# neggles/neurosis

Hardware: AMD Instinct MI355X
Metric: train images/sec (node) SDXL 1024^2 (higher is better)
Workload: dtype bf16

## Files before the change

### neurosis_amd/csrc/conv_halo.h

```cpp
#pragma once
#include <type_traits>

#ifdef NK_HALO_STAMPS
__device__ unsigned long long nk_halo_stamp_buf[8 * 8192];
__device__ unsigned long long nk_halo_kstep_buf[3 * 16 * 20 * 5];
#define CH_KSTAMP(t, ph) do { const int w_ = tid >> 6; if ((tid & 63) == 0 && (w_ == 0 || w_ == 4 || w_ == 6) && blockIdx.x >= 2048 && blockIdx.x < 2048 + 16 && (t) < 20) \
    nk_halo_kstep_buf[((((w_ == 0 ? 0 : (w_ == 4 ? 1 : 2)) * 16 + (blockIdx.x - 2048)) * 20 + (t)) * 5) + (ph)] = __builtin_amdgcn_s_memtime(); } while (0)
extern "C" int nk_debug_halo_ksteps(unsigned long long* host_out) {
  return hipMemcpyFromSymbol(host_out, HIP_SYMBOL(nk_halo_kstep_buf), sizeof(nk_halo_kstep_buf)) == hipSuccess ? 0 : 1;
}
#define CH_STAMP(slot) do { if (tid == 0 && blockIdx.x < 8192) nk_halo_stamp_buf[blockIdx.x * 8 + (slot)] = __builtin_amdgcn_s_memtime(); } while (0)
#define CH_STAMP_RT(slot) do { if (tid == 0 && blockIdx.x < 8192) nk_halo_stamp_buf[blockIdx.x * 8 + (slot)] = __builtin_amdgcn_s_memrealtime(); } while (0)
extern "C" int nk_debug_halo_stamps(unsigned long long* host_out, int nwg) {
  return hipMemcpyFromSymbol(host_out, HIP_SYMBOL(nk_halo_stamp_buf), (size_t)nwg * 8 * sizeof(unsigned long long)) == hipSuccess ? 0 : 1;
}
#else
#define CH_STAMP(slot)
#define CH_STAMP_RT(slot)
#define CH_KSTAMP(t, ph)
#endif
#define CH_TW 32
#define CH_HW (CH_TW + 2)
#define CH_BSTAGE 20480
#define CH_NS 3
#define CH_BSTAGE_DEEP 16384
#define CH_NS_DEEP 4
template <int BN_> struct HaloRing {
#ifdef NK_HALO_FIRE_IN_M
  static constexpr bool DEEP = false;
#else
  static constexpr bool DEEP = BN_ == 128;
#endif
  static constexpr int BST = DEEP ? CH_BSTAGE_DEEP : CH_BSTAGE;
  static constexpr int NS = DEEP ? CH_NS_DEEP : CH_NS;
  static constexpr int AHEAD = 2;
#ifdef NK_HALO_NO_PROD
  static constexpr bool PROD = false;
#else
  static constexpr bool PROD = DEEP;
#endif
  static constexpr bool FIRE_IN_R = DEEP && !PROD;
  static constexpr int THREADS = PROD ? 768 : 512;
  static constexpr int WAVES_PER_SIMD = PROD ? 3 : 2;
};
#define CH_NPROD_W 3
#define CH_NBW 6

template <int MI>
struct HaloGeom {
  static constexpr int TH = 2 * MI;
  static constexpr int RPW = MI / 2;
  static constexpr int HPX = (TH + 2) * CH_HW;
  static constexpr int HPIECES = ((HPX + 7) / 8 + 1) & ~1;
  static constexpr int HBUF = HPIECES * 1024;
  static constexpr int HPW = HPIECES / 2;
  static constexpr int SMEM = 2 * HBUF + CH_NS * CH_BSTAGE;
  static constexpr int SMEM_DEEP = 2 * HBUF + CH_NS_DEEP * CH_BSTAGE_DEEP;
  template <int BN_> static constexpr int smem() { return HaloRing<BN_>::DEEP ? SMEM_DEEP : SMEM; }
};
constexpr int ch_count(int NPH, int LAST, int t) { return t > LAST ? 0 : (NPH + LAST - t) / (LAST + 1); }
constexpr int ch_start(int NPH, int LAST, int t) { int s = 0; for (int u = 0; u < t; ++u) s += ch_count(NPH, LAST, u); return s; }

template <int BN_, int NBW = CH_NBW>
struct HaloWeights {
  static constexpr int NPC = BN_ / 8;
  static constexpr int NPW = (NPC + NBW - 1) / NBW;
  const bf16_t* rp[NPW];
  bool ok[NPW];
  __device__ __forceinline__ static int pieces(int wave) { return wave >= NBW ? 0 : (wave + NBW * (NPW - 1) < NPC ? NPW : NPW - 1); }
  __device__ __forceinline__ void init(const bf16_t* Wt, long ld, int Cout, int n0, int wave, int lane) {
#pragma unroll
    for (int i = 0; i < NPW; ++i) {
      const int pc = wave + NBW * i;
      const int row = pc * 8 + (lane >> 3);
      const int chunk = (lane & 7) ^ (lane >> 3);
      ok[i] = wave < NBW && pc < NPC && n0 + row < Cout;
      rp[i] = Wt + (long)(n0 + (ok[i] ? row : 0)) * ld + chunk * 8;
    }
  }
  __device__ __forceinline__ void fire_next(bool live, long adv, char* img, int wave) {
    const bf16_t* zp = (const bf16_t*)nk_zero_page;
#pragma unroll
    for (int i = 0; i < NPW; ++i) {
      if (wave + NBW * i < NPC)
        __builtin_amdgcn_global_load_lds((nk_gptr)((live && ok[i]) ? rp[i] : zp), (nk_lptr)(img + (wave + NBW * i) * 1024), 16, 0, 0);
      rp[i] += adv;
    }
  }
};

template <int BN_, int MI, int STATS>
__global__ __launch_bounds__(HaloRing<BN_>::THREADS, HaloRing<BN_>::WAVES_PER_SIMD) void nk_conv3x3_halo_kernel(const NkGemmParams p) {
  extern __shared__ __attribute__((aligned(16))) char smem[];
  using G = HaloGeom<MI>;
  using R = HaloRing<BN_>;
  constexpr int HN = BN_ / 2, NJ = HN / 16;
  constexpr int RPW = G::RPW, HPW = G::HPW, HBUF = G::HBUF;
  constexpr int HLAST = 6;
  const int tid = threadIdx.x, lane = tid & 63;
  const int wave = __builtin_amdgcn_readfirstlane(tid >> 6);
  const int grp = wave >> 2, wq = wave & 3;
  constexpr bool PROD = HaloRing<BN_>::PROD;
  const bool hwave = !PROD && wave >= CH_NBW;
  CH_STAMP(0);

  const int H = p.ga.H, W = p.ga.W, Cin = p.ga.C, Cout = p.N;
  const int txn = (W + CH_TW - 1) / CH_TW, tyn = (H + G::TH - 1) / G::TH;
  const int per_img = txn * tyn;
  const int ntm = p.halo_nb * per_img, ntn = (Cout + BN_ - 1) / BN_;
  const int nwg = gridDim.x, bid = blockIdx.x;
  const int q8 = nwg >> 3, r8 = nwg & 7, xcd = bid & 7;
  const int wg = (xcd < r8 ? xcd * (q8 + 1) : r8 * (q8 + 1) + (xcd - r8) * q8) + (bid >> 3);
  constexpr int GM = 16;
  const int per_group = GM * ntn;
  const int group = wg / per_group;
  const int first_m = group * GM;
  const int gm = min(GM, ntm - first_m);
  const int in_group = wg - group * per_group;
  const int nt = in_group / gm;
  const int mt = first_m + (in_group - nt * gm);
  const int n0 = nt * BN_;
  const int img = mt / per_img;
  const int trem = mt - img * per_img;
  const int tyi = trem / txn;
  const int y0 = tyi * G::TH, x0 = (trem - tyi * txn) * CH_TW;
  const int nslab = Cin >> 6, nk = nslab * 9;

  typedef __attribute__((address_space(3))) const char* lds_c;
  const unsigned lds0 = (unsigned)(size_t)(lds_c)smem;
  char* const ring = smem + 2 * HBUF;

  constexpr int HPP = PROD ? G::HPIECES : HPW;
  const int hw = PROD ? 0 : wave - CH_NBW;
  const int hp0 = hw * HPP * 8 + (lane >> 3);
  auto fire_halo = [&](int i, int slab, char* hbuf) {
    const int hp = hp0 + 8 * i;
    const int py = hp / CH_HW, px = hp - py * CH_HW;
    const int y = y0 - 1 + py, x = x0 - 1 + px;
    const bool v = hp < G::HPX && (unsigned)y < (unsigned)H && (unsigned)x < (unsigned)W;
    const int chunk = (lane & 7) ^ (hp & 7);
    const bf16_t* src = v ? p.A + ((long)((img * H + y) * W + x) * Cin + chunk * 8 + slab * 64) : (const bf16_t*)nk_zero_page;
    __builtin_amdgcn_global_load_lds((nk_gptr)src, (nk_lptr)(hbuf + (hw * HPP + i) * 1024), 16, 0, 0);
  };

  using WB = HaloWeights<BN_, PROD ? CH_NPROD_W : CH_NBW>;
  const int sw = PROD ? wave - 8 : wave;
  WB wb;
  if (!PROD || wave >= 8) wb.init(p.B, p.ldb, Cout, n0, sw, lane);
  const long adv_tap = Cin, adv_slab = 64 - 8l * Cin;
  const int s0 = p.k_rotate ? (xcd * nslab) >> 3 : 0;
  const long adv_wrap = 64 - 9l * Cin;
#define CH_BAR() __builtin_amdgcn_sched_barrier(0); __builtin_amdgcn_s_barrier(); __builtin_amdgcn_sched_barrier(0)
  if constexpr (PROD) {
    if (wave >= 8) {
      const int pw = wave - 8;
      const bool halo_wave = pw == CH_NPROD_W;
      const int npw = WB::pieces(pw);
      if (halo_wave) {
#pragma unroll
        for (int i = 0; i < HPP; ++i) fire_halo(i, s0, smem);
        asm volatile("s_waitcnt vmcnt(0)" ::: "memory");
      } else {
#pragma unroll
        for (int i = 0; i < WB::NPW; ++i) wb.rp[i] += s0 * 64;
        wb.fire_next(true, adv_tap, ring, pw);
        wb.fire_next(nk > 1, adv_tap, ring + R::BST, pw);
        if (npw == 6) asm volatile("s_waitcnt vmcnt(6)" ::: "memory");
        else asm volatile("s_waitcnt vmcnt(5)" ::: "memory");
      }
      CH_BAR();
      unsigned sn = R::AHEAD * R::BST;
      int t = 0, sl = s0;
      for (int s = 0; s < nslab; ++s) {
        char* const hnext = smem + ((s + 1) & 1) * HBUF;
        const bool more = s + 1 < nslab;
        const int sln = sl + 1 == nslab ? 0 : sl + 1;
        const long adv_end = sl + 1 == nslab ? adv_wrap : adv_slab;
        auto pstep = [&](auto tapc) {
          constexpr int tap = decltype(tapc)::value;
          constexpr int tap2 = (tap + 2) % 9;
          if (!halo_wave) wb.fire_next(t + 2 < nk, tap2 == 8 ? adv_end : adv_tap, ring + sn, pw);
          CH_BAR();
          if (halo_wave) {
            if (more) {
              constexpr int cnt = ch_count(HPP, HLAST, tap), st = ch_start(HPP, HLAST, tap);
#pragma unroll
              for (int i = 0; i < cnt; ++i) fire_halo(st + i, sln, hnext);
            }
            if (tap == 8) asm volatile("s_waitcnt vmcnt(0)" ::: "memory");
          } else {
            if (npw == 6) asm volatile("s_waitcnt vmcnt(6)" ::: "memory");
            else asm volatile("s_waitcnt vmcnt(5)" ::: "memory");
          }
          CH_BAR();
          sn += R::BST; if (sn == R::NS * R::BST) sn = 0;
          ++t;
        };
        pstep(std::integral_constant<int, 0>{}); pstep(std::integral_constant<int, 1>{}); pstep(std::integral_constant<int, 2>{});
        pstep(std::integral_constant<int, 3>{}); pstep(std::integral_constant<int, 4>{}); pstep(std::integral_constant<int, 5>{});
        pstep(std::integral_constant<int, 6>{}); pstep(std::integral_constant<int, 7>{}); pstep(std::integral_constant<int, 8>{});
        sl = sln;
      }
      asm volatile("s_waitcnt vmcnt(0)" ::: "memory");
      CH_BAR();
      return;
    }
  } else {
#pragma unroll
    for (int i = 0; i < WB::NPW; ++i) wb.rp[i] += s0 * 64;
    if (hwave) {
#pragma unroll
      for (int i = 0; i < HPW; ++i) fire_halo(i, s0, smem);
    } else {
      wb.fire_next(true, adv_tap, ring, wave);
      wb.fire_next(nk > 1, adv_tap, ring + R::BST, wave);
    }
  }

  FragG2<OP_KC, BN_, NJ> fb;
  fb.init(lds0 + 2 * HBUF, grp * HN, lane);
  const int hpl = wq * RPW * CH_HW + (lane & 15);
  const int cl4 = lane >> 4;
  const int g4 = lane >> 4;
  const int nb = n0 + grp * HN;
  float4_t acc[MI][NJ];
#pragma unroll
  for (int i = 0; i < MI; ++i)
#pragma unroll
    for (int j = 0; j < NJ; ++j) acc[i][j] = (float4_t){0.f, 0.f, 0.f, 0.f};
  bf16x8_t af[2 * MI], bfr[2 * NJ];

  const int nbw = PROD ? 0 : WB::pieces(wave);

  if constexpr (!PROD) {
    if (hwave) {
      asm volatile("s_waitcnt vmcnt(0)" ::: "memory");
    } else {
      if (nbw == 4) asm volatile("s_waitcnt vmcnt(4)" ::: "memory");
      else if (nbw == 3) asm volatile("s_waitcnt vmcnt(3)" ::: "memory");
      else asm volatile("s_waitcnt vmcnt(2)" ::: "memory");
    }
  }
  CH_BAR();
  CH_STAMP(1); CH_STAMP_RT(4);
  if (grp == 1) { CH_BAR(); }

  unsigned so = 0, sn = R::AHEAD * R::BST;
  int t = 0;
  int sl = s0;
  for (int s = 0; s < nslab; ++s) {
    const unsigned hcur = lds0 + (unsigned)(s & 1) * HBUF;
    char* const hnext = smem + ((s + 1) & 1) * HBUF;
    const bool more = s + 1 < nslab;
    const int sln = sl + 1 == nslab ? 0 : sl + 1;
    const long adv_end = sl + 1 == nslab ? adv_wrap : adv_slab;
    auto step = [&](auto tapc) {
      constexpr int tap = decltype(tapc)::value;
      constexpr int dy = tap / 3, dx = tap % 3;
      __builtin_amdgcn_sched_barrier(0);
      int hpv = hpl;
      asm volatile("" : "+v"(hpv));
      g2_read<OP_KC, BN_, NJ>(bfr, fb, so);
#pragma unroll
      for (int r = 0; r < RPW; ++r) {
        const int hp = hpv + (r + dy) * CH_HW + dx;
        const unsigned ar = (unsigned)(hp * 128 + ((cl4 ^ (hp & 7)) << 4));
        const unsigned a0 = hcur + ar, a1 = hcur + (ar ^ 64u);
        G2_RD128(af[2 * r], a0, 0);
        G2_RD128(af[2 * r + 1], a0, 2048);
        G2_RD128(af[MI + 2 * r], a1, 0);
        G2_RD128(af[MI + 2 * r + 1], a1, 2048);
      }
      if constexpr (PROD) {
      } else if (hwave) {
        if (more) {
          constexpr int cnt = ch_count(HPW, HLAST, tap), st = ch_start(HPW, HLAST, tap);
#pragma unroll
          for (int i = 0; i < cnt; ++i) fire_halo(st + i, sln, hnext);
        }
        if (tap == 8) asm volatile("s_waitcnt vmcnt(0)" ::: "memory");
      } else if constexpr (R::FIRE_IN_R) {
        constexpr int tap2 = (tap + 2) % 9;
        wb.fire_next(t + 2 < nk, tap2 == 8 ? adv_end : adv_tap, ring + sn, wave);
        if (nbw == 3) asm volatile("s_waitcnt vmcnt(3)" ::: "memory");
        else asm volatile("s_waitcnt vmcnt(2)" ::: "memory");
      } else {
        asm volatile("s_waitcnt vmcnt(0)" ::: "memory");
      }
      CH_KSTAMP(t, 4);
      CH_BAR();
      CH_KSTAMP(t, 0);
      asm volatile("s_waitcnt lgkmcnt(0)" ::: "memory");
      __builtin_amdgcn_sched_barrier(0);
      __builtin_amdgcn_s_setprio(1);
      if constexpr (!R::FIRE_IN_R && !PROD) {
        if (!hwave) {
          constexpr int tap2 = (tap + 2) % 9;
          wb.fire_next(t + 2 < nk, tap2 == 8 ? adv_end : adv_tap, ring + sn, wave);
        }
      }
      CH_KSTAMP(t, 1);
#pragma unroll
      for (int ks = 0; ks < 2; ++ks)
#pragma unroll
        for (int i = 0; i < MI; ++i)
#pragma unroll
          for (int j = 0; j < NJ; ++j)
            acc[i][j] = __builtin_amdgcn_mfma_f32_16x16x32_bf16(bfr[ks * NJ + j], af[ks * MI + i], acc[i][j], 0, 0, 0);
      __builtin_amdgcn_s_setprio(0);
      CH_KSTAMP(t, 2);
      CH_BAR();
      CH_KSTAMP(t, 3);
      so += R::BST; if (so == R::NS * R::BST) so = 0;
      sn += R::BST; if (sn == R::NS * R::BST) sn = 0;
      ++t;
    };
    step(std::integral_constant<int, 0>{}); step(std::integral_constant<int, 1>{}); step(std::integral_constant<int, 2>{});
    step(std::integral_constant<int, 3>{}); step(std::integral_constant<int, 4>{}); step(std::integral_constant<int, 5>{});
    step(std::integral_constant<int, 6>{}); step(std::integral_constant<int, 7>{}); step(std::integral_constant<int, 8>{});
    sl = sln;
  }
  if (grp == 0) { CH_BAR(); }
  asm volatile("s_waitcnt vmcnt(0)" ::: "memory");
  CH_STAMP(2); CH_STAMP_RT(5);

  int mrow[MI];
  bool mok[MI];
#pragma unroll
  for (int i = 0; i < MI; ++i) {
    const int y = y0 + wq * RPW + (i >> 1), x = x0 + (i & 1) * 16 + (lane & 15);
    mok[i] = y < H && x < W;
    mrow[i] = (img * H + y) * W + x;
  }
  bf16_t* const C = (bf16_t*)p.C;
  uint4_t res8[MI][NJ / 2 ? NJ / 2 : 1];
  uint2_t res4[MI];
  if (p.residual) {
#pragma unroll
    for (int i = 0; i < MI; ++i) {
#pragma unroll
      for (int h = 0; h < NJ / 2; ++h) {
        const int n = nb + h * 32 + (g4 & 1) * 16 + (g4 >> 1) * 8;
        res8[i][h] = (mok[i] && n < Cout) ? *(const uint4_t*)(p.residual + (long)mrow[i] * p.ldr + n) : (uint4_t){0u, 0u, 0u, 0u};
      }
      if constexpr (NJ & 1) {
        const int n = nb + (NJ - 1) * 16 + g4 * 4;
        res4[i] = (mok[i] && n < Cout) ? *(const uint2_t*)(p.residual + (long)mrow[i] * p.ldr + n) : (uint2_t){0u, 0u};
      }
    }
  }
  float cadd[NJ / 2][8], cadd4[4];
#pragma unroll
  for (int h = 0; h < NJ / 2; ++h) {
    const int n = nb + h * 32 + (g4 & 1) * 16 + (g4 >> 1) * 8;
#pragma unroll
    for (int e = 0; e < 8; ++e) cadd[h][e] = 0.f;
    if (n < Cout) {
      if (p.bias) {
        const float4_t b0 = *(const float4_t*)(p.bias + n), b1 = *(const float4_t*)(p.bias + n + 4);
        cadd[h][0] = b0[0]; cadd[h][1] = b0[1]; cadd[h][2] = b0[2]; cadd[h][3] = b0[3];
        cadd[h][4] = b1[0]; cadd[h][5] = b1[1]; cadd[h][6] = b1[2]; cadd[h][7] = b1[3];
      }
      if (p.rowvec) {
        float t[8];
        unpack8(*(const uint4_t*)(p.rowvec + (long)img * p.ld_rowvec + n), t);
#pragma unroll
        for (int e = 0; e < 8; ++e) cadd[h][e] += t[e];
      }
    }
  }
#pragma unroll
  for (int e = 0; e < 4; ++e) cadd4[e] = 0.f;
  if constexpr (NJ & 1) {
    const int n = nb + (NJ - 1) * 16 + g4 * 4;
    if (n < Cout) {
      if (p.bias) { const float4_t b = *(const float4_t*)(p.bias + n); cadd4[0] = b[0]; cadd4[1] = b[1]; cadd4[2] = b[2]; cadd4[3] = b[3]; }
      if (p.rowvec) {
        float t[4];
        unpack4(*(const uint2_t*)(p.rowvec + (long)img * p.ld_rowvec + n), t);
        cadd4[0] += t[0]; cadd4[1] += t[1]; cadd4[2] += t[2]; cadd4[3] += t[3];
      }
    }
  }

  float st8[NJ / 2 ? NJ / 2 : 1][8][2], st4[4][2];
  if constexpr (STATS) {
#pragma unroll
    for (int h = 0; h < NJ / 2; ++h)
#pragma unroll
      for (int e = 0; e < 8; ++e) { st8[h][e][0] = 0.f; st8[h][e][1] = 0.f; }
#pragma unroll
    for (int e = 0; e < 4; ++e) { st4[e][0] = 0.f; st4[e][1] = 0.f; }
  }
#pragma unroll
  for (int i = 0; i < MI; ++i) {
#pragma unroll
    for (int h = 0; h < NJ / 2; ++h) {
      float v[8];
#pragma unroll
      for (int r = 0; r < 4; ++r) {
        const float a_own = acc[i][2 * h][r], b_own = acc[i][2 * h + 1][r];
        auto sw = __builtin_amdgcn_permlane16_swap(__float_as_uint(a_own), __float_as_uint(b_own), false, false);
        v[r] = __uint_as_float(sw[0]);
        v[4 + r] = __uint_as_float(sw[1]);
      }
      const int n = nb + h * 32 + (g4 & 1) * 16 + (g4 >> 1) * 8;
#pragma unroll
      for (int e = 0; e < 8; ++e) v[e] += cadd[h][e];
      if (p.residual) {
        float tr[8];
        unpack8(res8[i][h], tr);
#pragma unroll
        for (int e = 0; e < 8; ++e) v[e] += tr[e];
      }
      const uint4_t packed = pack8(v);
      const bool ok = mok[i] && n < Cout;
      if (ok) *(uint4_t*)(C + (long)mrow[i] * p.ldc + n) = packed;
      if constexpr (STATS) {
        float q[8];
        unpack8(packed, q);
#pragma unroll
        for (int e = 0; e < 8; ++e) { const float x = ok ? q[e] : 0.f; st8[h][e][0] += x; st8[h][e][1] += x * x; }
      }
    }
    if constexpr (NJ & 1) {
      const int n = nb + (NJ - 1) * 16 + g4 * 4;
      float v[4] = {acc[i][NJ - 1][0] + cadd4[0], acc[i][NJ - 1][1] + cadd4[1], acc[i][NJ - 1][2] + cadd4[2], acc[i][NJ - 1][3] + cadd4[3]};
      if (p.residual) {
        float tr[4];
        unpack4(res4[i], tr);
        v[0] += tr[0]; v[1] += tr[1]; v[2] += tr[2]; v[3] += tr[3];
      }
      uint2_t o;
      o.x = pack2bf(v[0], v[1]);
      o.y = pack2bf(v[2], v[3]);
      const bool ok = mok[i] && n < Cout;
      if (ok) *(uint2_t*)(C + (long)mrow[i] * p.ldc + n) = o;
      if constexpr (STATS) {
        float q[4];
        unpack4(o, q);
#pragma unroll
        for (int e = 0; e < 4; ++e) { const float x = ok ? q[e] : 0.f; st4[e][0] += x; st4[e][1] += x * x; }
      }
    }
  }
  if constexpr (STATS) {
    __syncthreads();
    float* const cs = (float*)ring;
    auto lane16_sum = [](float x) {
      x += __builtin_bit_cast(float, __builtin_amdgcn_update_dpp(0, __builtin_bit_cast(int, x), 0xB1, 0xF, 0xF, true));
      x += __builtin_bit_cast(float, __builtin_amdgcn_update_dpp(0, __builtin_bit_cast(int, x), 0x4E, 0xF, 0xF, true));
      x += __builtin_bit_cast(float, __builtin_amdgcn_update_dpp(0, __builtin_bit_cast(int, x), 0x141, 0xF, 0xF, true));
      x += __builtin_bit_cast(float, __builtin_amdgcn_update_dpp(0, __builtin_bit_cast(int, x), 0x140, 0xF, 0xF, true));
      return x;
    };
#pragma unroll
    for (int h = 0; h < NJ / 2; ++h)
#pragma unroll
      for (int e = 0; e < 8; ++e)
#pragma unroll
        for (int k = 0; k < 2; ++k) {
          const float tot = lane16_sum(st8[h][e][k]);
          const int col = h * 32 + (g4 & 1) * 16 + (g4 >> 1) * 8 + e;
          if ((lane & 15) == 0) cs[(wave * HN + col) * 2 + k] = tot;
        }
    if constexpr (NJ & 1) {
#pragma unroll
      for (int e = 0; e < 4; ++e)
#pragma unroll
        for (int k = 0; k < 2; ++k) {
          const float tot = lane16_sum(st4[e][k]);
          const int col = (NJ - 1) * 16 + g4 * 4 + e;
          if ((lane & 15) == 0) cs[(wave * HN + col) * 2 + k] = tot;
        }
    }
    __syncthreads();
    const int cpg = Cout / p.stats_groups;
    const int ngt = BN_ / cpg;
    if (tid < 2 * ngt) {
      const int gi = tid >> 1, k = tid & 1;
      float a = 0.f;
      for (int cc = 0; cc < cpg; ++cc) {
        const int col = gi * cpg + cc;
        const int gh = col / HN, cl = col - gh * HN;
#pragma unroll
        for (int w4 = 0; w4 < 4; ++w4) a += cs[((gh * 4 + w4) * HN + cl) * 2 + k];
      }
      p.stats_part[((long)img * per_img + trem) * 2 * p.stats_groups + 2 * (n0 / cpg + gi) + k] = a;
    }
  }
#ifdef NK_HALO_STAMPS
  asm volatile("s_waitcnt vmcnt(0)" ::: "memory");
  CH_STAMP(3);
#endif
#undef CH_BAR
}

static bool halo_shape_ok(const NkGemmParams& p) {
  const NkGather& g = p.ga;
  if (!p.halo_nb || g.KW != 3 || p.K != 9 * g.C || g.rs != 1 || g.ks != 1 || g.div != 1 || g.off_h != -1 || g.off_w != -1) return false;
  if (g.Ho != g.H || g.Wo != g.W || (g.C & 63) || p.alpha != 1.0f || p.nbatch) return false;
  if (p.N % 160 && p.N % 128) return false;
  if ((p.N & 7) || (p.ldc & 7) || (p.residual && (p.ldr & 7))) return false;
  return true;
}
static int halo_bn(int N) { return N % 160 == 0 ? 160 : 128; }
static int halo_tile_rows(const NkGemmParams& p) {
  const NkGather& g = p.ga;
  const int bn = halo_bn(p.N);
  const long txn = (g.W + CH_TW - 1) / CH_TW;
  for (int th = 8; th >= 4; th -= 4) {
    const long tyn = (g.H + th - 1) / th;
    const long cover = txn * CH_TW * tyn * th;
    if (cover * 100 > (long)g.H * g.W * 115) continue;
    const long tiles = (long)p.halo_nb * txn * tyn * (p.N / bn);
    if (th == 8 && tiles < 224) continue;
    return th;
  }
  return 0;
}
static bool use_halo(const NkGemmParams& p, int amode, int bmode, int out_f32) {
  if (amode != OP_KCG || bmode != OP_KC || out_f32) return false;
  if (const char* e = getenv("NK_CONV_HALO")) if (e[0] == '0') return false;
  return halo_shape_ok(p) && halo_tile_rows(p) != 0;
}

template <int BN_, int MI, int STATS>
static int launch_halo_as(const NkGemmParams& p_in, hipStream_t stream) {
  NkGemmParams p = p_in;
  p.k_rotate = k_rotate_on(p.ga.C) ? 1 : 0;
  auto kern = nk_conv3x3_halo_kernel<BN_, MI, STATS>;
  nk_optin_lds((const void*)kern, HaloGeom<MI>::template smem<BN_>());
  const NkGather& g = p.ga;
  const long tiles = (long)p.halo_nb * ((g.W + CH_TW - 1) / CH_TW) * ((g.H + HaloGeom<MI>::TH - 1) / HaloGeom<MI>::TH) * (p.N / BN_);
  hipLaunchKernelGGL(kern, dim3((unsigned)tiles), dim3(HaloRing<BN_>::THREADS), HaloGeom<MI>::template smem<BN_>(), stream, p);
  if (BN_ == 160 && MI == 4) return nk_check_launch(STATS ? "nk_conv3x3_halo_kernel<160,8,stats=1>" : "nk_conv3x3_halo_kernel<160,8,stats=0>");
  if (BN_ == 160) return nk_check_launch(STATS ? "nk_conv3x3_halo_kernel<160,4,stats=1>" : "nk_conv3x3_halo_kernel<160,4,stats=0>");
  if (MI == 4) return nk_check_launch(STATS ? "nk_conv3x3_halo_kernel<128,8,stats=1>" : "nk_conv3x3_halo_kernel<128,8,stats=0>");
  return nk_check_launch(STATS ? "nk_conv3x3_halo_kernel<128,4,stats=1>" : "nk_conv3x3_halo_kernel<128,4,stats=0>");
}
template <int STATS>
static int launch_halo_s(const NkGemmParams& p, hipStream_t stream) {
  const int th = halo_tile_rows(p);
  const bool wide = halo_bn(p.N) == 160;
  if (th == 8) return wide ? launch_halo_as<160, 4, STATS>(p, stream) : launch_halo_as<128, 4, STATS>(p, stream);
  return wide ? launch_halo_as<160, 2, STATS>(p, stream) : launch_halo_as<128, 2, STATS>(p, stream);
}
static int launch_halo(const NkGemmParams& p, hipStream_t stream) {
  return p.stats_part ? launch_halo_s<1>(p, stream) : launch_halo_s<0>(p, stream);
}
static int halo_tiles_per_image(const NkGemmParams& p) {
  const int th = halo_tile_rows(p);
  if (!th) return 0;
  return ((p.ga.W + CH_TW - 1) / CH_TW) * ((p.ga.H + th - 1) / th);
}
```

Baseline: 25.81.

## Add self-pipelined single-group consumer loop for 8-row 128-column halo conv tile

For the producer-variant halo conv with 8-row tiles and 128 columns, the block drops from 12 to 8 waves. A single group of 4 consumer waves each covers all 128 columns, with the B-fragment LDS reads double-buffered against the MFMAs under explicit lgkmcnt waits. One barrier per tap is removed on the producer side. The epilogue is reorganised into lambdas so the consumer can process both column halves in sequence, with residual loads for the second half overlapped against the first. This is meant to hide LDS latency and cut per-tap synchronisation, at the cost of more accumulator registers per wave and fewer waves to cover latency.

Measured after the change: 25.90, median of 6. About the same (+0.4%).

```diff
diff --git a/neurosis_amd/csrc/conv_halo.h b/neurosis_amd/csrc/conv_halo.h
--- a/neurosis_amd/csrc/conv_halo.h
+++ b/neurosis_amd/csrc/conv_halo.h
@@ -25,7 +25,7 @@
 #define CH_NS 3
 #define CH_BSTAGE_DEEP 16384
 #define CH_NS_DEEP 4
-template <int BN_> struct HaloRing {
+template <int BN_, int MI_ = 2> struct HaloRing {
 #ifdef NK_HALO_FIRE_IN_M
   static constexpr bool DEEP = false;
 #else
@@ -40,8 +40,14 @@
   static constexpr bool PROD = DEEP;
 #endif
   static constexpr bool FIRE_IN_R = DEEP && !PROD;
-  static constexpr int THREADS = PROD ? 768 : 512;
-  static constexpr int WAVES_PER_SIMD = PROD ? 3 : 2;
+#ifdef NK_HALO_TWO_GROUP
+  static constexpr bool SP = false;
+#else
+  static constexpr bool SP = PROD && MI_ == 4;
+#endif
+  static constexpr int THREADS = SP ? 512 : (PROD ? 768 : 512);
+  static constexpr int WAVES_PER_SIMD = SP ? 2 : (PROD ? 3 : 2);
+  static constexpr int PW0 = SP ? 4 : 8;
 };
 #define CH_NPROD_W 3
 #define CH_NBW 6
@@ -89,18 +95,26 @@
   }
 };
 
+template <int R>
+__device__ __forceinline__ void halo_sp_read(bf16x8_t (&fa)[4], bf16x8_t (&fb)[8], const unsigned (&ra)[2], unsigned rb) {
+  if constexpr (R < 4) G2_RD128(fa[R], ra[R >> 1], (R & 1) * 2048);
+  else G2_RD128(fb[R - 4], rb, (R - 4) * 2048);
+}
+
 template <int BN_, int MI, int STATS>
-__global__ __launch_bounds__(HaloRing<BN_>::THREADS, HaloRing<BN_>::WAVES_PER_SIMD) void nk_conv3x3_halo_kernel(const NkGemmParams p) {
+__global__ __launch_bounds__((HaloRing<BN_, MI>::THREADS), (HaloRing<BN_, MI>::WAVES_PER_SIMD)) void nk_conv3x3_halo_kernel(const NkGemmParams p) {
   extern __shared__ __attribute__((aligned(16))) char smem[];
   using G = HaloGeom<MI>;
-  using R = HaloRing<BN_>;
+  using R = HaloRing<BN_, MI>;
   constexpr int HN = BN_ / 2, NJ = HN / 16;
   constexpr int RPW = G::RPW, HPW = G::HPW, HBUF = G::HBUF;
   constexpr int HLAST = 6;
   const int tid = threadIdx.x, lane = tid & 63;
   const int wave = __builtin_amdgcn_readfirstlane(tid >> 6);
   const int grp = wave >> 2, wq = wave & 3;
-  constexpr bool PROD = HaloRing<BN_>::PROD;
+  constexpr bool PROD = R::PROD;
+  constexpr bool SP = R::SP;
+  constexpr int PW0 = R::PW0;
   const bool hwave = !PROD && wave >= CH_NBW;
   CH_STAMP(0);
 
@@ -144,16 +158,16 @@
   };
 
   using WB = HaloWeights<BN_, PROD ? CH_NPROD_W : CH_NBW>;
-  const int sw = PROD ? wave - 8 : wave;
+  const int sw = PROD ? wave - PW0 : wave;
   WB wb;
-  if (!PROD || wave >= 8) wb.init(p.B, p.ldb, Cout, n0, sw, lane);
+  if (!PROD || wave >= PW0) wb.init(p.B, p.ldb, Cout, n0, sw, lane);
   const long adv_tap = Cin, adv_slab = 64 - 8l * Cin;
   const int s0 = p.k_rotate ? (xcd * nslab) >> 3 : 0;
   const long adv_wrap = 64 - 9l * Cin;
 #define CH_BAR() __builtin_amdgcn_sched_barrier(0); __builtin_amdgcn_s_barrier(); __builtin_amdgcn_sched_barrier(0)
   if constexpr (PROD) {
-    if (wave >= 8) {
-      const int pw = wave - 8;
+    if (wave >= PW0) {
+      const int pw = wave - PW0;
       const bool halo_wave = pw == CH_NPROD_W;
       const int npw = WB::pieces(pw);
       if (halo_wave) {
@@ -180,7 +194,8 @@
           constexpr int tap = decltype(tapc)::value;
           constexpr int tap2 = (tap + 2) % 9;
           if (!halo_wave) wb.fire_next(t + 2 < nk, tap2 == 8 ? adv_end : adv_tap, ring + sn, pw);
-          CH_BAR();
+          CH_KSTAMP(t, 1);
+          if constexpr (!SP) { CH_BAR(); }
           if (halo_wave) {
             if (more) {
               constexpr int cnt = ch_count(HPP, HLAST, tap), st = ch_start(HPP, HLAST, tap);
@@ -192,7 +207,9 @@
             if (npw == 6) asm volatile("s_waitcnt vmcnt(6)" ::: "memory");
             else asm volatile("s_waitcnt vmcnt(5)" ::: "memory");
           }
+          CH_KSTAMP(t, 4);
           CH_BAR();
+          CH_KSTAMP(t + 1, 0);
           sn += R::BST; if (sn == R::NS * R::BST) sn = 0;
           ++t;
         };
@@ -217,17 +234,107 @@
     }
   }
 
-  FragG2<OP_KC, BN_, NJ> fb;
-  fb.init(lds0 + 2 * HBUF, grp * HN, lane);
+  constexpr int NJA = SP ? 2 * NJ : NJ;
   const int hpl = wq * RPW * CH_HW + (lane & 15);
   const int cl4 = lane >> 4;
   const int g4 = lane >> 4;
-  const int nb = n0 + grp * HN;
-  float4_t acc[MI][NJ];
+  float4_t acc[MI][NJA];
 #pragma unroll
   for (int i = 0; i < MI; ++i)
 #pragma unroll
-    for (int j = 0; j < NJ; ++j) acc[i][j] = (float4_t){0.f, 0.f, 0.f, 0.f};
+    for (int j = 0; j < NJA; ++j) acc[i][j] = (float4_t){0.f, 0.f, 0.f, 0.f};
+  if constexpr (SP) {
+    static_assert(MI == 4 && NJ == 4, "the self-pipelined loop is written for the 8-row 128-column tile");
+    __builtin_amdgcn_s_setprio(1);
+    FragG2<OP_KC, BN_, NJA> fbs;
+    fbs.init(lds0 + 2 * HBUF, 0, lane);
+    bf16x8_t fA[2][MI], fB[2][NJA];
+    unsigned rA[RPW], rB;
+    unsigned nA1[RPW];
+    auto tap_addr = [&](auto tapc, unsigned hb) {
+      constexpr int tap = decltype(tapc)::value, dy = tap / 3, dx = tap % 3;
+      int hpv = hpl;
+      asm volatile("" : "+v"(hpv));
+#pragma unroll
+      for (int r = 0; r < RPW; ++r) {
+        const int hp = hpv + (r + dy) * CH_HW + dx;
+        const unsigned ar = (unsigned)(hp * 128 + ((cl4 ^ (hp & 7)) << 4));
+        rA[r] = hb + ar;
+        nA1[r] = hb + (ar ^ 64u);
+      }
+    };
+    auto rd = [&](auto par_tag, auto r_tag) { halo_sp_read<decltype(r_tag)::value>(fA[decltype(par_tag)::value], fB[decltype(par_tag)::value], rA, rB); };
+    auto column = [&](auto cur_tag, auto j_tag) {
+      constexpr int CUR = decltype(cur_tag)::value, j = decltype(j_tag)::value, NXT = 1 - CUR;
+      constexpr int allow = j == 0 ? NJA - 1 : (NJA - 1 - j) + 2 * (j - 1);
+      static_assert(allow <= 15, "lgkmcnt is a 4-bit counter");
+      if constexpr (j == 0)
+        asm volatile("s_waitcnt lgkmcnt(%5)" : "+v"(fA[CUR][0]), "+v"(fA[CUR][1]), "+v"(fA[CUR][2]), "+v"(fA[CUR][3]), "+v"(fB[CUR][0]) : "n"(allow));
+      else
+        asm volatile("s_waitcnt lgkmcnt(%1)" : "+v"(fB[CUR][j]) : "n"(allow));
+      __builtin_amdgcn_sched_barrier(0);
+      constexpr bool ISSUE = j >= 1 && j <= 6;
+      acc[0][j] = __builtin_amdgcn_mfma_f32_16x16x32_bf16(fB[CUR][j], fA[CUR][0], acc[0][j], 0, 0, 0);
+      if constexpr (ISSUE) rd(std::integral_constant<int, NXT>{}, std::integral_constant<int, ISSUE ? 2 * (j - 1) : 0>{});
+      acc[1][j] = __builtin_amdgcn_mfma_f32_16x16x32_bf16(fB[CUR][j], fA[CUR][1], acc[1][j], 0, 0, 0);
+      __builtin_amdgcn_sched_barrier(0);
+      acc[2][j] = __builtin_amdgcn_mfma_f32_16x16x32_bf16(fB[CUR][j], fA[CUR][2], acc[2][j], 0, 0, 0);
+      if constexpr (ISSUE) rd(std::integral_constant<int, NXT>{}, std::integral_constant<int, ISSUE ? 2 * (j - 1) + 1 : 0>{});
+      acc[3][j] = __builtin_amdgcn_mfma_f32_16x16x32_bf16(fB[CUR][j], fA[CUR][3], acc[3][j], 0, 0, 0);
+      __builtin_amdgcn_sched_barrier(0);
+    };
+    auto columns_1_7 = [&](auto cur_tag) {
+      column(cur_tag, std::integral_constant<int, 1>{}); column(cur_tag, std::integral_constant<int, 2>{}); column(cur_tag, std::integral_constant<int, 3>{});
+      column(cur_tag, std::integral_constant<int, 4>{}); column(cur_tag, std::integral_constant<int, 5>{}); column(cur_tag, std::integral_constant<int, 6>{});
+      column(cur_tag, std::integral_constant<int, 7>{});
+    };
+
+    CH_BAR();
+    CH_STAMP(1); CH_STAMP_RT(4);
+    unsigned so = 0;
+    tap_addr(std::integral_constant<int, 0>{}, lds0);
+    rB = fbs.a[0];
+    rd(std::integral_constant<int, 0>{}, std::integral_constant<int, 0>{}); rd(std::integral_constant<int, 0>{}, std::integral_constant<int, 1>{});
+    rd(std::integral_constant<int, 0>{}, std::integral_constant<int, 2>{}); rd(std::integral_constant<int, 0>{}, std::integral_constant<int, 3>{});
+    rd(std::integral_constant<int, 0>{}, std::integral_constant<int, 4>{}); rd(std::integral_constant<int, 0>{}, std::integral_constant<int, 5>{});
+    rd(std::integral_constant<int, 0>{}, std::integral_constant<int, 6>{}); rd(std::integral_constant<int, 0>{}, std::integral_constant<int, 7>{});
+    rd(std::integral_constant<int, 0>{}, std::integral_constant<int, 8>{}); rd(std::integral_constant<int, 0>{}, std::integral_constant<int, 9>{});
+    rd(std::integral_constant<int, 0>{}, std::integral_constant<int, 10>{}); rd(std::integral_constant<int, 0>{}, std::integral_constant<int, 11>{});
+    asm volatile("s_waitcnt lgkmcnt(0)" : "+v"(fA[0][0]), "+v"(fA[0][1]), "+v"(fA[0][2]), "+v"(fA[0][3]), "+v"(fB[0][0]), "+v"(fB[0][1]), "+v"(fB[0][2]),
+                 "+v"(fB[0][3]), "+v"(fB[0][4]), "+v"(fB[0][5]), "+v"(fB[0][6]), "+v"(fB[0][7]));
+    __builtin_amdgcn_sched_barrier(0);
+    int t = 0;
+    for (int s = 0; s < nslab; ++s) {
+      const unsigned hcur = lds0 + (unsigned)(s & 1) * HBUF, hoth = lds0 + (unsigned)((s + 1) & 1) * HBUF;
+      auto step = [&](auto tapc) {
+        constexpr int tap = decltype(tapc)::value, ntap = (tap + 1) % 9;
+        CH_KSTAMP(t, 0);
+        (void)t;
+#pragma unroll
+        for (int r = 0; r < RPW; ++r) rA[r] = nA1[r];
+        rB = fbs.a[1] + so;
+        column(std::integral_constant<int, 0>{}, std::integral_constant<int, 0>{});
+        columns_1_7(std::integral_constant<int, 0>{});
+        column(std::integral_constant<int, 1>{}, std::integral_constant<int, 0>{});
+        CH_BAR();
+        so += R::BST; if (so == R::NS * R::BST) so = 0;
+        tap_addr(std::integral_constant<int, ntap>{}, tap == 8 ? hoth : hcur);
+        rB = fbs.a[0] + so;
+        __builtin_amdgcn_sched_barrier(0);
+        columns_1_7(std::integral_constant<int, 1>{});
+        ++t;
+      };
+      step(std::integral_constant<int, 0>{}); step(std::integral_constant<int, 1>{}); step(std::integral_constant<int, 2>{});
+      step(std::integral_constant<int, 3>{}); step(std::integral_constant<int, 4>{}); step(std::integral_constant<int, 5>{});
+      step(std::integral_constant<int, 6>{}); step(std::integral_constant<int, 7>{}); step(std::integral_constant<int, 8>{});
+    }
+    asm volatile("s_waitcnt lgkmcnt(0)" ::: "memory");
+    __builtin_amdgcn_s_setprio(0);
+    CH_BAR();
+    CH_STAMP(2); CH_STAMP_RT(5);
+  } else {
+  FragG2<OP_KC, BN_, NJ> fb;
+  fb.init(lds0 + 2 * HBUF, grp * HN, lane);
   bf16x8_t af[2 * MI], bfr[2 * NJ];
 
   const int nbw = PROD ? 0 : WB::pieces(wave);
@@ -323,6 +430,7 @@
   if (grp == 0) { CH_BAR(); }
   asm volatile("s_waitcnt vmcnt(0)" ::: "memory");
   CH_STAMP(2); CH_STAMP_RT(5);
+  }
 
   int mrow[MI];
   bool mok[MI];
@@ -333,83 +441,90 @@
     mrow[i] = (img * H + y) * W + x;
   }
   bf16_t* const C = (bf16_t*)p.C;
-  uint4_t res8[MI][NJ / 2 ? NJ / 2 : 1];
-  uint2_t res4[MI];
-  if (p.residual) {
-#pragma unroll
-    for (int i = 0; i < MI; ++i) {
+  float* const cs = (float*)ring;
+  auto lane16_sum = [](float x) {
+    x += __builtin_bit_cast(float, __builtin_amdgcn_update_dpp(0, __builtin_bit_cast(int, x), 0xB1, 0xF, 0xF, true));
+    x += __builtin_bit_cast(float, __builtin_amdgcn_update_dpp(0, __builtin_bit_cast(int, x), 0x4E, 0xF, 0xF, true));
+    x += __builtin_bit_cast(float, __builtin_amdgcn_update_dpp(0, __builtin_bit_cast(int, x), 0x141, 0xF, 0xF, true));
+    x += __builtin_bit_cast(float, __builtin_amdgcn_update_dpp(0, __builtin_bit_cast(int, x), 0x140, 0xF, 0xF, true));
+    return x;
+  };
+  struct Res { uint4_t r8[NJ / 2 ? NJ / 2 : 1]; uint2_t r4; };
+  struct Add { float c8[NJ / 2 ? NJ / 2 : 1][8], c4[4]; };
+  struct Sums { float s8[NJ / 2 ? NJ / 2 : 1][8][2], s4[4][2]; };
+  auto res_load = [&](const int nb, const int i, Res& rs) {
+    if (p.residual) {
 #pragma unroll
       for (int h = 0; h < NJ / 2; ++h) {
         const int n = nb + h * 32 + (g4 & 1) * 16 + (g4 >> 1) * 8;
-        res8[i][h] = (mok[i] && n < Cout) ? *(const uint4_t*)(p.residual + (long)mrow[i] * p.ldr + n) : (uint4_t){0u, 0u, 0u, 0u};
+        rs.r8[h] = (mok[i] && n < Cout) ? *(const uint4_t*)(p.residual + (long)mrow[i] * p.ldr + n) : (uint4_t){0u, 0u, 0u, 0u};
       }
       if constexpr (NJ & 1) {
         const int n = nb + (NJ - 1) * 16 + g4 * 4;
-        res4[i] = (mok[i] && n < Cout) ? *(const uint2_t*)(p.residual + (long)mrow[i] * p.ldr + n) : (uint2_t){0u, 0u};
-      }
-    }
-  }
-  float cadd[NJ / 2][8], cadd4[4];
-#pragma unroll
-  for (int h = 0; h < NJ / 2; ++h) {
-    const int n = nb + h * 32 + (g4 & 1) * 16 + (g4 >> 1) * 8;
-#pragma unroll
-    for (int e = 0; e < 8; ++e) cadd[h][e] = 0.f;
-    if (n < Cout) {
-      if (p.bias) {
-        const float4_t b0 = *(const float4_t*)(p.bias + n), b1 = *(const float4_t*)(p.bias + n + 4);
-        cadd[h][0] = b0[0]; cadd[h][1] = b0[1]; cadd[h][2] = b0[2]; cadd[h][3] = b0[3];
-        cadd[h][4] = b1[0]; cadd[h][5] = b1[1]; cadd[h][6] = b1[2]; cadd[h][7] = b1[3];
-      }
-      if (p.rowvec) {
-        float t[8];
-        unpack8(*(const uint4_t*)(p.rowvec + (long)img * p.ld_rowvec + n), t);
-#pragma unroll
-        for (int e = 0; e < 8; ++e) cadd[h][e] += t[e];
-      }
-    }
-  }
-#pragma unroll
-  for (int e = 0; e < 4; ++e) cadd4[e] = 0.f;
-  if constexpr (NJ & 1) {
-    const int n = nb + (NJ - 1) * 16 + g4 * 4;
-    if (n < Cout) {
-      if (p.bias) { const float4_t b = *(const float4_t*)(p.bias + n); cadd4[0] = b[0]; cadd4[1] = b[1]; cadd4[2] = b[2]; cadd4[3] = b[3]; }
-      if (p.rowvec) {
-        float t[4];
-        unpack4(*(const uint2_t*)(p.rowvec + (long)img * p.ld_rowvec + n), t);
-        cadd4[0] += t[0]; cadd4[1] += t[1]; cadd4[2] += t[2]; cadd4[3] += t[3];
-      }
-    }
-  }
-
-  float st8[NJ / 2 ? NJ / 2 : 1][8][2], st4[4][2];
-  if constexpr (STATS) {
+        rs.r4 = (mok[i] && n < Cout) ? *(const uint2_t*)(p.residual + (long)mrow[i] * p.ldr + n) : (uint2_t){0u, 0u};
+      }
+    }
+  };
+  auto add_load = [&](const int nb, Add& ad) {
+#pragma unroll
+    for (int h = 0; h < NJ / 2; ++h) {
+      const int n = nb + h * 32 + (g4 & 1) * 16 + (g4 >> 1) * 8;
+#pragma unroll
+      for (int e = 0; e < 8; ++e) ad.c8[h][e] = 0.f;
+      if (n < Cout) {
+        if (p.bias) {
+          const float4_t b0 = *(const float4_t*)(p.bias + n), b1 = *(const float4_t*)(p.bias + n + 4);
+          ad.c8[h][0] = b0[0]; ad.c8[h][1] = b0[1]; ad.c8[h][2] = b0[2]; ad.c8[h][3] = b0[3];
+          ad.c8[h][4] = b1[0]; ad.c8[h][5] = b1[1]; ad.c8[h][6] = b1[2]; ad.c8[h][7] = b1[3];
+        }
+        if (p.rowvec) {
+          float t[8];
+          unpack8(*(const uint4_t*)(p.rowvec + (long)img * p.ld_rowvec + n), t);
+#pragma unroll
+          for (int e = 0; e < 8; ++e) ad.c8[h][e] += t[e];
+        }
+      }
+    }
+#pragma unroll
+    for (int e = 0; e < 4; ++e) ad.c4[e] = 0.f;
+    if constexpr (NJ & 1) {
+      const int n = nb + (NJ - 1) * 16 + g4 * 4;
+      if (n < Cout) {
+        if (p.bias) { const float4_t b = *(const float4_t*)(p.bias + n); ad.c4[0] = b[0]; ad.c4[1] = b[1]; ad.c4[2] = b[2]; ad.c4[3] = b[3]; }
+        if (p.rowvec) {
+          float t[4];
+          unpack4(*(const uint2_t*)(p.rowvec + (long)img * p.ld_rowvec + n), t);
+          ad.c4[0] += t[0]; ad.c4[1] += t[1]; ad.c4[2] += t[2]; ad.c4[3] += t[3];
+        }
+      }
+    }
+  };
+  auto sums_zero = [&](Sums& su) {
 #pragma unroll
     for (int h = 0; h < NJ / 2; ++h)
 #pragma unroll
-      for (int e = 0; e < 8; ++e) { st8[h][e][0] = 0.f; st8[h][e][1] = 0.f; }
-#pragma unroll
-    for (int e = 0; e < 4; ++e) { st4[e][0] = 0.f; st4[e][1] = 0.f; }
-  }
-#pragma unroll
-  for (int i = 0; i < MI; ++i) {
+      for (int e = 0; e < 8; ++e) { su.s8[h][e][0] = 0.f; su.s8[h][e][1] = 0.f; }
+#pragma unroll
+    for (int e = 0; e < 4; ++e) { su.s4[e][0] = 0.f; su.s4[e][1] = 0.f; }
+  };
+  auto row_block = [&](auto jb_tag, const int nb, const int i, const Res& rs, const Add& ad, Sums& su) {
+    constexpr int JB = decltype(jb_tag)::value;
 #pragma unroll
     for (int h = 0; h < NJ / 2; ++h) {
       float v[8];
 #pragma unroll
       for (int r = 0; r < 4; ++r) {
-        const float a_own = acc[i][2 * h][r], b_own = acc[i][2 * h + 1][r];
+        const float a_own = acc[i][JB + 2 * h][r], b_own = acc[i][JB + 2 * h + 1][r];
         auto sw = __builtin_amdgcn_permlane16_swap(__float_as_uint(a_own), __float_as_uint(b_own), false, false);
         v[r] = __uint_as_float(sw[0]);
         v[4 + r] = __uint_as_float(sw[1]);
       }
       const int n = nb + h * 32 + (g4 & 1) * 16 + (g4 >> 1) * 8;
 #pragma unroll
-      for (int e = 0; e < 8; ++e) v[e] += cadd[h][e];
+      for (int e = 0; e < 8; ++e) v[e] += ad.c8[h][e];
       if (p.residual) {
         float tr[8];
-        unpack8(res8[i][h], tr);
+        unpack8(rs.r8[h], tr);
 #pragma unroll
         for (int e = 0; e < 8; ++e) v[e] += tr[e];
       }
@@ -420,15 +535,15 @@
         float q[8];
         unpack8(packed, q);
 #pragma unroll
-        for (int e = 0; e < 8; ++e) { const float x = ok ? q[e] : 0.f; st8[h][e][0] += x; st8[h][e][1] += x * x; }
+        for (int e = 0; e < 8; ++e) { const float x = ok ? q[e] : 0.f; su.s8[h][e][0] += x; su.s8[h][e][1] += x * x; }
       }
     }
     if constexpr (NJ & 1) {
       const int n = nb + (NJ - 1) * 16 + g4 * 4;
-      float v[4] = {acc[i][NJ - 1][0] + cadd4[0], acc[i][NJ - 1][1] + cadd4[1], acc[i][NJ - 1][2] + cadd4[2], acc[i][NJ - 1][3] + cadd4[3]};
+      float v[4] = {acc[i][JB + NJ - 1][0] + ad.c4[0], acc[i][JB + NJ - 1][1] + ad.c4[1], acc[i][JB + NJ - 1][2] + ad.c4[2], acc[i][JB + NJ - 1][3] + ad.c4[3]};
       if (p.residual) {
         float tr[4];
-        unpack4(res4[i], tr);
+        unpack4(rs.r4, tr);
         v[0] += tr[0]; v[1] += tr[1]; v[2] += tr[2]; v[3] += tr[3];
       }
       uint2_t o;
@@ -440,40 +555,67 @@
         float q[4];
         unpack4(o, q);
 #pragma unroll
-        for (int e = 0; e < 4; ++e) { const float x = ok ? q[e] : 0.f; st4[e][0] += x; st4[e][1] += x * x; }
-      }
-    }
-  }
-  if constexpr (STATS) {
-    __syncthreads();
-    float* const cs = (float*)ring;
-    auto lane16_sum = [](float x) {
-      x += __builtin_bit_cast(float, __builtin_amdgcn_update_dpp(0, __builtin_bit_cast(int, x), 0xB1, 0xF, 0xF, true));
-      x += __builtin_bit_cast(float, __builtin_amdgcn_update_dpp(0, __builtin_bit_cast(int, x), 0x4E, 0xF, 0xF, true));
-      x += __builtin_bit_cast(float, __builtin_amdgcn_update_dpp(0, __builtin_bit_cast(int, x), 0x141, 0xF, 0xF, true));
-      x += __builtin_bit_cast(float, __builtin_amdgcn_update_dpp(0, __builtin_bit_cast(int, x), 0x140, 0xF, 0xF, true));
-      return x;
-    };
+        for (int e = 0; e < 4; ++e) { const float x = ok ? q[e] : 0.f; su.s4[e][0] += x; su.s4[e][1] += x * x; }
+      }
+    }
+  };
+  auto sums_out = [&](const int fw, const Sums& su) {
 #pragma unroll
     for (int h = 0; h < NJ / 2; ++h)
 #pragma unroll
       for (int e = 0; e < 8; ++e)
 #pragma unroll
         for (int k = 0; k < 2; ++k) {
-          const float tot = lane16_sum(st8[h][e][k]);
+          const float tot = lane16_sum(su.s8[h][e][k]);
           const int col = h * 32 + (g4 & 1) * 16 + (g4 >> 1) * 8 + e;
-          if ((lane & 15) == 0) cs[(wave * HN + col) * 2 + k] = tot;
+          if ((lane & 15) == 0) cs[(fw * HN + col) * 2 + k] = tot;
         }
     if constexpr (NJ & 1) {
 #pragma unroll
       for (int e = 0; e < 4; ++e)
 #pragma unroll
         for (int k = 0; k < 2; ++k) {
-          const float tot = lane16_sum(st4[e][k]);
+          const float tot = lane16_sum(su.s4[e][k]);
           const int col = (NJ - 1) * 16 + g4 * 4 + e;
-          if ((lane & 15) == 0) cs[(wave * HN + col) * 2 + k] = tot;
+          if ((lane & 15) == 0) cs[(fw * HN + col) * 2 + k] = tot;
         }
     }
+  };
+  if constexpr (SP) {
+    Res r0[MI], r1[MI];
+    Add a0, a1;
+    Sums su;
+#pragma unroll
+    for (int i = 0; i < MI; ++i) res_load(n0, i, r0[i]);
+    add_load(n0, a0);
+    add_load(n0 + HN, a1);
+    if constexpr (STATS) sums_zero(su);
+#pragma unroll
+    for (int i = 0; i < MI; ++i) {
+      row_block(std::integral_constant<int, 0>{}, n0, i, r0[i], a0, su);
+      res_load(n0 + HN, i, r1[i]);
+    }
+    if constexpr (STATS) { sums_out(wq, su); sums_zero(su); }
+#pragma unroll
+    for (int i = 0; i < MI; ++i) row_block(std::integral_constant<int, NJ>{}, n0 + HN, i, r1[i], a1, su);
+    if constexpr (STATS) sums_out(4 + wq, su);
+  } else {
+    const int nb = n0 + grp * HN;
+    Res rs[MI];
+    Add ad;
+    Sums su;
+#pragma unroll
+    for (int i = 0; i < MI; ++i) res_load(nb, i, rs[i]);
+    add_load(nb, ad);
+    if constexpr (STATS) sums_zero(su);
+#pragma unroll
+    for (int i = 0; i < MI; ++i) row_block(std::integral_constant<int, 0>{}, nb, i, rs[i], ad, su);
+    if constexpr (STATS) {
+      __syncthreads();
+      sums_out(wave, su);
+    }
+  }
+  if constexpr (STATS) {
     __syncthreads();
     const int cpg = Cout / p.stats_groups;
     const int ngt = BN_ / cpg;
@@ -533,7 +675,7 @@
   nk_optin_lds((const void*)kern, HaloGeom<MI>::template smem<BN_>());
   const NkGather& g = p.ga;
   const long tiles = (long)p.halo_nb * ((g.W + CH_TW - 1) / CH_TW) * ((g.H + HaloGeom<MI>::TH - 1) / HaloGeom<MI>::TH) * (p.N / BN_);
-  hipLaunchKernelGGL(kern, dim3((unsigned)tiles), dim3(HaloRing<BN_>::THREADS), HaloGeom<MI>::template smem<BN_>(), stream, p);
+  hipLaunchKernelGGL(kern, dim3((unsigned)tiles), dim3(HaloRing<BN_, MI>::THREADS), HaloGeom<MI>::template smem<BN_>(), stream, p);
   if (BN_ == 160 && MI == 4) return nk_check_launch(STATS ? "nk_conv3x3_halo_kernel<160,8,stats=1>" : "nk_conv3x3_halo_kernel<160,8,stats=0>");
   if (BN_ == 160) return nk_check_launch(STATS ? "nk_conv3x3_halo_kernel<160,4,stats=1>" : "nk_conv3x3_halo_kernel<160,4,stats=0>");
   if (MI == 4) return nk_check_launch(STATS ? "nk_conv3x3_halo_kernel<128,8,stats=1>" : "nk_conv3x3_halo_kernel<128,8,stats=0>");
```
